# jinggqu/NextGen-UIA

Hardware: AMD Instinct MI355X
Metric: images/sec fwd+bwd BiomedCLIP+Mona bs=256 (higher is better)
Workload: dtype bf16

## Files before the change

nextgen-uia_amd/csrc/attention_bwd.hip:

```cpp
#include "uia_common.h"
#include "uia_kernels.h"

#ifdef ABWD_STAMPS
__device__ unsigned long long uia_abwd_stamps[8 * 8];
extern "C" int uia_abwd_read_stamps(unsigned long long* host) {
    return (int)hipMemcpyFromSymbol(host, HIP_SYMBOL(uia_abwd_stamps), sizeof(uia_abwd_stamps));
}
#define STAMP() __builtin_amdgcn_s_memtime()
#endif

namespace {

typedef __attribute__((ext_vector_type(4))) short s16x4;
typedef __attribute__((ext_vector_type(8))) short s16x8;

__device__ __forceinline__ void glds16(const char* gsrc, char* lds_wave_base) {
    const unsigned dst_u = __builtin_amdgcn_readfirstlane((unsigned)(uintptr_t)(__attribute__((address_space(3))) char*)lds_wave_base);
    unsigned keep;
    asm volatile("s_mov_b32 %0, m0\n\ts_mov_b32 m0, %2\n\ts_nop 0\n\tglobal_load_lds_dwordx4 %1, off\n\ts_mov_b32 m0, %0"
                 : "=&s"(keep) : "v"(gsrc), "s"(dst_u) : "memory");
}
__device__ __forceinline__ void glds4(const char* gsrc, char* lds_wave_base) {
    const unsigned dst_u = __builtin_amdgcn_readfirstlane((unsigned)(uintptr_t)(__attribute__((address_space(3))) char*)lds_wave_base);
    unsigned keep;
// ... 227 lines not shown
                qT[dt] = tr_pair(Qb + off, Qb + off + 16 * 128);
            }
        }
        const bool full_q = p.mask_kind == UIA_MASK_NONE && 32 * u + 32 <= L;
#pragma unroll
        for (int a = 0; a < KTW; ++a) {
            const int kt = wave + BWD_WAVES * a;
            if (kt < LT) {
                const int key = 16 * kt + li;
                bf16x8 pf, sf;
                f32x4 s[2], dp[2];
#pragma unroll
                for (int hq = 0; hq < 2; ++hq) {
                    s[hq] = mma(qf[hq][0], kf[a][0], f32x4{0.f, 0.f, 0.f, 0.f});
                    dp[hq] = mma(gf[hq][0], vf[a][0], f32x4{0.f, 0.f, 0.f, 0.f});
                }
#pragma unroll
                for (int hq = 0; hq < 2; ++hq) {
                    s[hq] = mma(qf[hq][1], kf[a][1], s[hq]);
                    dp[hq] = mma(gf[hq][1], vf[a][1], dp[hq]);
                }
#ifdef ABWD_NO_VALU
                if (true) {
#pragma unroll
                    for (int e = 0; e < 8; ++e) { pf[e] = (bf16_t)s[e >> 2][e & 3]; sf[e] = (bf16_t)dp[e >> 2][e & 3]; }
                } else
#endif
                if (full_q && 16 * kt + 16 <= L) {
#pragma unroll
                    for (int hq = 0; hq < 2; ++hq)
#pragma unroll
                        for (int r = 0; r < 4; ++r) {
                            const float pv = __builtin_amdgcn_exp2f(fmaf(s[hq][r], sc, -ls[hq][r]));
                            const float dsv = pv * fmaf(dp[hq][r], p.scale, -dl[hq][r]);
                            pf[4 * hq + r] = (bf16_t)pv;
                            sf[4 * hq + r] = (bf16_t)dsv;
                        }
                } else if (p.mask_kind != UIA_MASK_CAUSAL && 32 * u + 32 <= L) {
                    const bool key_ok = key < klen;
#pragma unroll
                    for (int hq = 0; hq < 2; ++hq)
#pragma unroll
                        for (int r = 0; r < 4; ++r) {
                            const float pe = __builtin_amdgcn_exp2f(fmaf(s[hq][r], sc, -ls[hq][r]));
                            const float pv = key_ok ? pe : 0.f;
                            const float dsv = pv * fmaf(dp[hq][r], p.scale, -dl[hq][r]);
                            pf[4 * hq + r] = (bf16_t)pv;
                            sf[4 * hq + r] = (bf16_t)dsv;
                        }
                } else {
#pragma unroll
                    for (int hq = 0; hq < 2; ++hq)
#pragma unroll
                        for (int r = 0; r < 4; ++r) {
                            const int qrow = 32 * u + 16 * hq + 4 * g + r;
                            const int kmax = p.mask_kind == UIA_MASK_CAUSAL ? (qrow < klen - 1 ? qrow : klen - 1) : klen - 1;
                            const bool ok = qrow < L && key <= kmax;
                            const float pv = ok ? __builtin_amdgcn_exp2f(fmaf(s[hq][r], sc, -ls[hq][r])) : 0.f;
                            const float dsv = pv * fmaf(dp[hq][r], p.scale, -dl[hq][r]);
                            pf[4 * hq + r] = (bf16_t)pv;
                            sf[4 * hq + r] = (bf16_t)dsv;
                        }
                }
                {
                    typedef __attribute__((ext_vector_type(4))) __bf16 bf16x4_t;
                    char* rowp = dST + key * 64;
                    const int sw = (key >> 1) & 7;
                    *(bf16x4_t*)(rowp + (((0 + g) ^ sw) << 3)) = bf16x4_t{sf[0], sf[1], sf[2], sf[3]};
                    *(bf16x4_t*)(rowp + (((4 + g) ^ sw) << 3)) = bf16x4_t{sf[4], sf[5], sf[6], sf[7]};
                }
#ifndef ABWD_NO_DVDK
#pragma unroll
                for (int dt = 0; dt < 4; ++dt) {
                    if constexpr (LAZY_T) {
                        const int off = trow * 128 + (((2 * dt + (pp >> 1)) ^ tsw) << 4) + 8 * (pp & 1);
                        gT[dt] = tr_pair(Gb + off, Gb + off + 16 * 128);
                        qT[dt] = tr_pair(Qb + off, Qb + off + 16 * 128);
                    }
                    dVt[a][dt] = __builtin_amdgcn_mfma_f32_16x16x32_bf16(gT[dt], pf, dVt[a][dt], 0, 0, 0);
                    dKt[a][dt] = __builtin_amdgcn_mfma_f32_16x16x32_bf16(qT[dt], sf, dKt[a][dt], 0, 0, 0);
                }
#endif
            }
        }
        }
#ifdef ABWD_STAMPS
        asm volatile("s_waitcnt lgkmcnt(0)" ::: "memory");
        const unsigned long long st3 = STAMP();
#endif
#ifndef ABWD_NO_DQ
        if (u > 0) {
#else
        if (false) {
#endif
            const int hq = wave >> 2, dt = wave & 3;
            f32x4 dq = f32x4{0.f, 0.f, 0.f, 0.f}, dq1 = f32x4{0.f, 0.f, 0.f, 0.f};
            const int ch = 2 * dt + (pp >> 1);
            const int c8 = 4 * hq + pp;
            auto dq_step = [&](int kbk, f32x4 accq) {
                const char* klo = Ks + (32 * kbk + nrow) * 128 + ((ch ^ nsw_lo) << 4) + 8 * (pp & 1);
                const char* khi = Ks + (32 * kbk + nrow + 4) * 128 + ((ch ^ nsw_hi) << 4) + 8 * (pp & 1);
                const char* slo = dSTr + (32 * kbk + nrow) * 64 + ((c8 ^ nsw_lo) << 3);
                const char* shi = dSTr + (32 * kbk + nrow + 4) * 64 + ((c8 ^ nsw_hi) << 3);
                return __builtin_amdgcn_mfma_f32_16x16x32_bf16(tr_pair(klo, khi), tr_pair(slo, shi), accq, 0, 0, 0);
            };
#pragma unroll 1
            for (int kbk = 0; kbk < NP; kbk += 2) {
                dq = dq_step(kbk, dq);
                if (kbk + 1 < NP) dq1 = dq_step(kbk + 1, dq1);
            }
            dq_hold = dq + dq1;
        }
#ifdef ABWD_STAMPS
        asm volatile("" :: "v"(dq_hold));
        const unsigned long long st4 = STAMP();
        st_acc[0] += st1 - st0; st_acc[1] += st2 - st1; st_acc[2] += st3 - st2; st_acc[3] += st4 - st3;
#endif
    }
#ifndef ABWD_NO_DQ
    store_dq(NP - 1);
#endif
#pragma unroll
    for (int a = 0; a < KTW; ++a) {
        const int kt = wave + BWD_WAVES * a;
        const int key = 16 * kt + li;
        if (kt < LT && key < L) {
            bf16_t* krow = (bf16_t*)p.dk + (row0 + key) * p.ld_dqkv + (size_t)h * 64 + 4 * g;
            bf16_t* vrow = (bf16_t*)p.dv + (row0 + key) * p.ld_dqkv + (size_t)h * 64 + 4 * g;
            const size_t kbo = ((size_t)(2 * h) * (size_t)p.dqkv_kb_rows + row0 + key) * 32 + 4 * g, kbp = (size_t)p.dqkv_kb_rows * 32;
#pragma unroll
            for (int dt = 0; dt < 4; ++dt) {
                store4(p.dqkv_kb_rows ? (bf16_t*)p.dk + kbo + (dt >> 1) * kbp + 16 * (dt & 1) : krow + 16 * dt, dKt[a][dt]);
                store4(p.dqkv_kb_rows ? (bf16_t*)p.dv + kbo + (dt >> 1) * kbp + 16 * (dt & 1) : vrow + 16 * dt, dVt[a][dt]);
            }
        }
    }
#ifdef ABWD_STAMPS
    if (blockIdx.x == 1500 && lane == 0) {
        unsigned long long* o = uia_abwd_stamps + wave * 8;
        o[0] = st_acc[0]; o[1] = st_acc[1]; o[2] = st_acc[2]; o[3] = st_acc[3]; o[4] = st_pro; o[5] = STAMP() - st_begin;
    }
#endif
}

struct ctrue { static constexpr bool value = true; };
struct cfalse { static constexpr bool value = false; };
template <int V> struct cint { static constexpr int value = V; };

#ifndef ABWD_ORDER17
#define ABWD_ORDER17 1
#endif
constexpr bool ORDER17 = ABWD_ORDER17 != 0;

template <int NW, bool VLDS, bool OLDS>
__global__ __launch_bounds__(64 * NW, (NW + 3) / 4) void attn_bwd_units_kernel(const UiaAttnParams p) {
    extern __shared__ __attribute__((aligned(16))) char smem[];
    constexpr int KVS = VLDS ? 4096 : 2048;
    constexpr bool KGLOBAL = false, QGLOBAL = false;
    const int L = p.L;
    const int LT = (L + 15) >> 4, NP = (LT + 1) >> 1;
    char* QGg = smem;
    char* KVg = QGg + LT * 4096;
    char* STg = KVg + LT * KVS;
    int* queue = (int*)(STg + LT * 128);
    char* OBg = STg + LT * 128 + 64;
    float* lseb = (float*)(OBg + LT * 2048);
    const lptr QG = (lptr)smem, KV = QG + LT * 4096, ST = KV + LT * KVS;

    const int tid = threadIdx.x, lane = tid & 63;
    const int wave = __builtin_amdgcn_readfirstlane(tid >> 6);
#ifdef ABWD_STAMPS
    const unsigned long long st_begin = STAMP();
    unsigned long long st_u[2] = {0, 0}, st_n[2] = {0, 0}, st_pro = 0, st_loop = 0, st_iter = 0;
#endif
    const int b = blockIdx.x / p.H, h = blockIdx.x - b * p.H;
    const size_t row0 = (size_t)b * L;
    const size_t rs = (size_t)p.ld_qkv * 2, rso = (size_t)p.lddo * 2, rsO = (size_t)p.ldo * 2;
    const char* qb = (const char*)p.q + (row0 * p.ld_qkv + (size_t)h * 64) * 2;
    const char* kb = (const char*)p.k + (row0 * p.ld_qkv + (size_t)h * 64) * 2;
    const char* vb = (const char*)p.v + (row0 * p.ld_qkv + (size_t)h * 64) * 2;
    const char* gb = (const char*)p.dout + (row0 * p.lddo + (size_t)h * 64) * 2;
    const char* ob = (const char*)p.out + (row0 * p.ldo + (size_t)h * 64) * 2;
    const int li = lane & 15, g = lane >> 4;
    int klen = L;
    if (p.mask_kind == UIA_MASK_KEYPAD && p.keylen) { klen = p.keylen[b]; klen = klen < 1 ? 1 : (klen > L ? L : klen); }
    klen = __builtin_amdgcn_readfirstlane(klen);
    const bool causal = p.mask_kind == UIA_MASK_CAUSAL;

    if constexpr (OLDS) {
        const int npieces = 2 * LT;
        for (int q = wave; q < npieces; q += NW) {
            const int r = 8 * q + (lane >> 3);
            const int gr = r < L ? r : L - 1;
            const int c = ((lane & 7) ^ (r & 6)) * 16;
            const int t = q >> 1, half = (q & 1) * 1024;
            glds16(gb + gr * rso + c, QGg + t * 4096 + 2048 + half);
            glds16(p.out_kb_rows ? (const char*)p.out + (((size_t)(2 * h + (c >> 6)) * (size_t)p.out_kb_rows + row0 + gr) << 6) + (c & 63) : ob + gr * rsO + c,
                   OBg + q * 1024);
        }
        for (int i = wave; i * 64 < 16 * LT; i += NW) {
            int r = 64 * i + lane;
            r = r < L ? r : L - 1;
            glds4((const char*)(p.lse + ((size_t)b * p.H + h) * L + r), (char*)(lseb + 64 * i));
        }
        for (int q = wave; q < npieces; q += NW) {
            const int r = 8 * q + (lane >> 3);
            const int gr = r < L ? r : L - 1;
            const int c = ((lane & 7) ^ (r & 6)) * 16;
            const int t = q >> 1, half = (q & 1) * 1024;
            glds16(kb + gr * rs + c, KVg + t * KVS + half);
            glds16(qb + gr * rs + c, QGg + t * 4096 + half);
            if (VLDS) glds16(vb + gr * rs + c, KVg + t * KVS + 2048 + half);
        }
        if (tid == 0) *queue = 0;
        const int nk = ((npieces - wave + NW - 1) / NW) * (VLDS ? 3 : 2);
        if (nk >= 9) asm volatile("s_waitcnt vmcnt(9)" ::: "memory");
        else if (nk >= 6) asm volatile("s_waitcnt vmcnt(6)" ::: "memory");
        else asm volatile("s_waitcnt vmcnt(0)" ::: "memory");
        __syncthreads();
        for (int r0 = 0; r0 < 16 * LT; r0 += NW * 8) {
            const int r = r0 + (tid >> 3), part = tid & 7;
            if (r < 16 * LT) {
                const int off = (r & 15) * 128 + ((part ^ (r & 6)) << 4);
                const bf16x8 gv = *(const bf16x8*)(QGg + (r >> 4) * 4096 + 2048 + off);
                const bf16x8 ovv = *(const bf16x8*)(OBg + (r >> 4) * 2048 + off);
                float d = 0.f;
#pragma unroll
                for (int e = 0; e < 8; ++e) d = fmaf((float)gv[e], (float)ovv[e], d);
                d += __builtin_bit_cast(float, __builtin_amdgcn_update_dpp(0, __builtin_bit_cast(int, d), 0xB1, 0xF, 0xF, false));
                d += __builtin_bit_cast(float, __builtin_amdgcn_update_dpp(0, __builtin_bit_cast(int, d), 0x4E, 0xF, 0xF, false));
                d += __builtin_bit_cast(float, __builtin_amdgcn_update_dpp(0, __builtin_bit_cast(int, d), 0x141, 0xF, 0xF, false));
                if (part == 0) {
                    float* st = (float*)(STg + (r >> 4) * 128) + (r & 15);
                    st[0] = r < L ? lseb[r] * 1.44269504088896341f : 0.f;
                    st[16] = r < L ? -d : 0.f;
                }
            }
        }
        asm volatile("s_waitcnt vmcnt(0)" ::: "memory");
        __syncthreads();
    } else
    {
        constexpr int RPP = NW * 8, MAXP = (288 + RPP - 1) / RPP;
        bf16x8 gv[MAXP], ov[MAXP];
        float lv[MAXP];
#pragma unroll
        for (int i = 0; i < MAXP; ++i) {
            const int r = i * RPP + (tid >> 3), part = tid & 7;
            if (i * RPP < 16 * LT) {
                const int gr = r < L ? r : L - 1;
                gv[i] = *(const bf16x8*)(gb + gr * rso + part * 16);
                ov[i] = *(const bf16x8*)(p.out_kb_rows ? (const char*)p.out + (((size_t)(2 * h + (part >> 2)) * (size_t)p.out_kb_rows + row0 + gr) << 6) + (part & 3) * 16
                                                       : ob + gr * rsO + part * 16);
                lv[i] = p.lse[((size_t)b * p.H + h) * L + gr];
            }
        }
        const int npieces = 2 * LT;
        for (int q = wave; q < npieces; q += NW) {
            const int r = 8 * q + (lane >> 3);
            const int gr = r < L ? r : L - 1;
            const int c = ((lane & 7) ^ (r & 6)) * 16;
            const int t = q >> 1, half = (q & 1) * 1024;
            glds16(kb + gr * rs + c, KVg + t * KVS + half);
            glds16(qb + gr * rs + c, QGg + t * 4096 + half);
            glds16(gb + gr * rso + c, QGg + t * 4096 + 2048 + half);
            if (VLDS) glds16(vb + gr * rs + c, KVg + t * KVS + 2048 + half);
        }
        if (tid == 0) *queue = 0;
#pragma unroll
        for (int i = 0; i < MAXP; ++i) {
            const int r = i * RPP + (tid >> 3), part = tid & 7;
            if (i * RPP < 16 * LT) {
                float d = 0.f;
#pragma unroll
                for (int e = 0; e < 8; ++e) d = fmaf((float)gv[i][e], (float)ov[i][e], d);
                d += __builtin_bit_cast(float, __builtin_amdgcn_update_dpp(0, __builtin_bit_cast(int, d), 0xB1, 0xF, 0xF, false));
                d += __builtin_bit_cast(float, __builtin_amdgcn_update_dpp(0, __builtin_bit_cast(int, d), 0x4E, 0xF, 0xF, false));
                d += __builtin_bit_cast(float, __builtin_amdgcn_update_dpp(0, __builtin_bit_cast(int, d), 0x141, 0xF, 0xF, false));
                if (part == 0 && r < 16 * LT) {
                    float* st = (float*)(STg + (r >> 4) * 128) + (r & 15);
                    st[0] = r < L ? lv[i] * 1.44269504088896341f : 0.f;
                    st[16] = r < L ? -d : 0.f;
                }
            }
        }
        asm volatile("s_waitcnt vmcnt(0)" ::: "memory");
        __syncthreads();
    }
#ifdef ABWD_STAMPS
    st_pro = STAMP() - st_begin;
#endif

    const float sc = p.scale * 1.44269504088896341f;
    const int offR0 = li * 128 + ((g ^ (li & 6)) << 4);
    const int offR1 = offR0 ^ 64;
    const int qq = li >> 2, pp = li & 3;
    const int trow = 4 * g + qq;
    const int tsw = trow & 6;
    int toff[4];
#pragma unroll
    for (int dt = 0; dt < 4; ++dt) toff[dt] = trow * 128 + (((2 * dt + (pp >> 1)) ^ tsw) << 4) + 8 * (pp & 1);
    const f32x4 zero4 = f32x4{0.f, 0.f, 0.f, 0.f};

    for (;;) {
        int unit = 0;
        if (lane == 0) unit = atomicAdd(queue, 1);
        unit = __builtin_amdgcn_readfirstlane(unit);
        if (unit >= 2 * LT) break;
#ifdef ABWD_STAMPS
        const unsigned long long st_u0 = STAMP();
#endif
        bool is_key = unit < LT;
        int tile = is_key ? unit : unit - LT;
        if (ORDER17 && LT == 17) {
            if (unit < 3) { is_key = true; tile = unit; }
            else if (unit < 10) { is_key = false; tile = unit - 3; }
            else if (unit < 24) { is_key = true; tile = unit - 7; }
            else { is_key = false; tile = unit - 17; }
        }
        if (is_key) {
            const int kt = tile;
#include "attention_bwd_key_unit.inc"
        } else {
            const int qt = tile;
#include "attention_bwd_qry_unit.inc"
        }
#ifdef ABWD_STAMPS
        st_u[is_key ? 0 : 1] += STAMP() - st_u0; st_n[is_key ? 0 : 1] += 1;
#endif
    }
#ifdef ABWD_STAMPS
    if (blockIdx.x == 1500 && lane == 0 && wave < 8) {
        unsigned long long* o = uia_abwd_stamps + wave * 8;
        o[0] = st_pro; o[1] = st_u[0]; o[2] = st_u[1]; o[3] = st_n[0]; o[4] = st_n[1]; o[5] = STAMP() - st_begin; o[6] = st_loop; o[7] = st_iter;
    }
#endif
}
template <int NW>
__global__ __launch_bounds__(64 * NW, 2) void attn_bwd_persist_kernel(const UiaAttnParams p, const int nheads) {
    extern __shared__ __attribute__((aligned(16))) char smem[];
    constexpr bool VLDS = true, KGLOBAL = true, QGLOBAL = true;
    constexpr int KVS = 4096;
    const int L = p.L;
    const int LT = (L + 15) >> 4, NP = (LT + 1) >> 1;
    char* QGg = smem;
    char* KVg = QGg + LT * 4096;
    char* STg = KVg + LT * KVS;
    char* OBg = STg + 2 * LT * 128;
    float* lseb = (float*)(OBg + LT * 2048);
    int* ctr = (int*)(lseb + ((16 * LT + 63) & ~63));
    const lptr QG = (lptr)smem, KV = QG + LT * 4096;
    const lptr STb = KV + LT * KVS;
    lptr ST = STb;

    const int tid = threadIdx.x, lane = tid & 63;
    const int wave = __builtin_amdgcn_readfirstlane(tid >> 6);
#ifdef ABWD_STAMPS
    const unsigned long long st_begin = STAMP();
    unsigned long long st_u[2] = {0, 0}, st_n[2] = {0, 0}, st_pro = 0, st_loop = 0, st_iter = 0, st_bar = 0;
#endif
    const int li = lane & 15, g = lane >> 4;
    const bool causal = p.mask_kind == UIA_MASK_CAUSAL;
    const size_t rs = (size_t)p.ld_qkv * 2, rso = (size_t)p.lddo * 2, rsO = (size_t)p.ldo * 2;
    const float sc = p.scale * 1.44269504088896341f;
    const int offR0 = li * 128 + ((g ^ (li & 6)) << 4);
    const int offR1 = offR0 ^ 64;
    const int qq = li >> 2, pp = li & 3;
    const int trow = 4 * g + qq;
    const int tsw = trow & 6;
    int toff[4];
#pragma unroll
    for (int dt = 0; dt < 4; ++dt) toff[dt] = trow * 128 + (((2 * dt + (pp >> 1)) ^ tsw) << 4) + 8 * (pp & 1);
    const f32x4 zero4 = f32x4{0.f, 0.f, 0.f, 0.f};

    int b = 0, h = 0, klen = L;
    size_t row0 = 0;
    const char *qb = nullptr, *kb = nullptr, *vb = nullptr, *gb = nullptr;
    auto set_head = [&](int n) {
        b = n / p.H; h = n - b * p.H;
        row0 = (size_t)b * L;
        qb = (const char*)p.q + (row0 * p.ld_qkv + (size_t)h * 64) * 2;
        kb = (const char*)p.k + (row0 * p.ld_qkv + (size_t)h * 64) * 2;
        vb = (const char*)p.v + (row0 * p.ld_qkv + (size_t)h * 64) * 2;
        gb = (const char*)p.dout + (row0 * p.lddo + (size_t)h * 64) * 2;
        klen = L;
        if (p.mask_kind == UIA_MASK_KEYPAD && p.keylen) { klen = p.keylen[b]; klen = klen < 1 ? 1 : (klen > L ? L : klen); }
        klen = __builtin_amdgcn_readfirstlane(klen);
    };
    auto stage_qg = [&](int n) {
        const int nb = n / p.H, nh = n - nb * p.H;
        const size_t nrow0 = (size_t)nb * L;
        const char* nq = (const char*)p.q + (nrow0 * p.ld_qkv + (size_t)nh * 64) * 2;
        const char* ng = (const char*)p.dout + (nrow0 * p.lddo + (size_t)nh * 64) * 2;
        const char* no = (const char*)p.out + (nrow0 * p.ldo + (size_t)nh * 64) * 2;
        for (int q = wave; q < 2 * LT; q += NW) {
            const int r = 8 * q + (lane >> 3);
            const int gr = r < L ? r : L - 1;
            const int c = ((lane & 7) ^ (r & 6)) * 16;
            const int t = q >> 1, half = (q & 1) * 1024;
            glds16(nq + gr * rs + c, QGg + t * 4096 + half);
            glds16(ng + gr * rso + c, QGg + t * 4096 + 2048 + half);
            glds16(p.out_kb_rows ? (const char*)p.out + (((size_t)(2 * nh + (c >> 6)) * (size_t)p.out_kb_rows + nrow0 + gr) << 6) + (c & 63) : no + gr * rsO + c,
                   OBg + q * 1024);
        }
        for (int i = wave; i * 64 < 16 * LT; i += NW) {
            int r = 64 * i + lane;
            r = r < L ? r : L - 1;
            glds4((const char*)(p.lse + ((size_t)nb * p.H + nh) * L + r), (char*)(lseb + 64 * i));
        }
    };
    auto stage_kv = [&]() {
        for (int q = wave; q < 2 * LT; q += NW) {
            const int r = 8 * q + (lane >> 3);
            const int gr = r < L ? r : L - 1;
            const int c = ((lane & 7) ^ (r & 6)) * 16;
            const int t = q >> 1, half = (q & 1) * 1024;
            glds16(kb + gr * rs + c, KVg + t * KVS + half);
            glds16(vb + gr * rs + c, KVg + t * KVS + 2048 + half);
        }
    };
    auto delta = [&](char* st_dst) {
        for (int r0 = 0; r0 < 16 * LT; r0 += NW * 8) {
            const int r = r0 + (tid >> 3), part = tid & 7;
            if (r < 16 * LT) {
                const int off = (r & 15) * 128 + ((part ^ (r & 6)) << 4);
                const bf16x8 gv = *(const bf16x8*)(QGg + (r >> 4) * 4096 + 2048 + off);
                const bf16x8 ovv = *(const bf16x8*)(OBg + (r >> 4) * 2048 + off);
                float d = 0.f;
#pragma unroll
                for (int e = 0; e < 8; ++e) d = fmaf((float)gv[e], (float)ovv[e], d);
                d += __builtin_bit_cast(float, __builtin_amdgcn_update_dpp(0, __builtin_bit_cast(int, d), 0xB1, 0xF, 0xF, false));
                d += __builtin_bit_cast(float, __builtin_amdgcn_update_dpp(0, __builtin_bit_cast(int, d), 0x4E, 0xF, 0xF, false));
                d += __builtin_bit_cast(float, __builtin_amdgcn_update_dpp(0, __builtin_bit_cast(int, d), 0x141, 0xF, 0xF, false));
                if (part == 0) {
                    float* st = (float*)(st_dst + (r >> 4) * 128) + (r & 15);
                    st[0] = r < L ? lseb[r] * 1.44269504088896341f : 0.f;
                    st[16] = r < L ? -d : 0.f;
                }
            }
        }
    };
    auto next_unit = [&](int which) {
        int u = 0;
        if (lane == 0) u = atomicAdd(ctr + which, 1);
        return __builtin_amdgcn_readfirstlane(u);
    };
    auto seam = [&]() {
        asm volatile("s_waitcnt vmcnt(0)" ::: "memory");
        __syncthreads();
    };

    int n = blockIdx.x;
    if (n >= nheads) return;
    stage_qg(n);
    if (tid == 0) { ctr[0] = 0; ctr[1] = 0; }
    seam();
    delta(STg);
    __syncthreads();
    set_head(n);
#ifdef ABWD_STAMPS
    st_pro = STAMP() - st_begin;
#endif
    int cur = 0;
    for (;;) {
        ST = STb + cur * (LT * 128);
        stage_kv();
        for (;;) {
            const int kt = next_unit(0);
            if (kt >= LT) break;
#ifdef ABWD_STAMPS
            const unsigned long long st_u0 = STAMP();
#endif
#include "attention_bwd_key_unit.inc"
// ... 28 lines not shown
#endif
        seam();
        delta(STg + (cur ^ 1) * (LT * 128));
        if (tid == 0) { ctr[0] = 0; ctr[1] = 0; }
        __syncthreads();
#ifdef ABWD_STAMPS
        st_bar += STAMP() - st_b1;
#endif
        n = nn;
        set_head(n);
        cur ^= 1;
    }
#ifdef ABWD_STAMPS
    if (blockIdx.x == 100 && lane == 0 && wave < 8) {
        unsigned long long* o = uia_abwd_stamps + wave * 8;
        o[0] = st_pro; o[1] = st_u[0]; o[2] = st_u[1]; o[3] = st_n[0]; o[4] = st_n[1]; o[5] = STAMP() - st_begin; o[6] = st_bar; o[7] = st_iter;
    }
#endif
}
__host__ __device__ constexpr int persist_lds_bytes(int LT) {
    return LT * 8192 + 2 * LT * 128 + LT * 2048 + ((16 * LT + 63) / 64) * 256 + 64 + 1024;
}
constexpr int PERSIST_LT_MAX = 15;

__host__ __device__ constexpr int units_lds_bytes(int LT, bool vlds, bool olds = false) {
    const int kvs = vlds ? 4096 : 2048, need = kvs + 64 - LT * 128;
    return LT * 4096 + LT * kvs + LT * 128 + 64 + (olds ? LT * 2048 + ((16 * LT + 63) / 64) * 256 + 1024 : (need > 1024 ? need : 1024));
}
constexpr int OLDS_LT_MAX = 15;


__global__ __launch_bounds__(256) void attn_bwd_f32_kernel(const UiaAttnParams p) {
    extern __shared__ __attribute__((aligned(16))) char smem[];
    const int L = p.L;
    float* A = (float*)smem;
    float* Bm = A + (size_t)L * 64;
    float* lse = Bm + (size_t)L * 64;
    float* delta = lse + L;
    const int tid = threadIdx.x;
    const int b = blockIdx.x / p.H, h = blockIdx.x - b * p.H;
    const size_t row0 = (size_t)b * L;
    const float* qb = (const float*)p.q + row0 * p.ld_qkv + (size_t)h * 64;
    const float* kb = (const float*)p.k + row0 * p.ld_qkv + (size_t)h * 64;
    const float* vb = (const float*)p.v + row0 * p.ld_qkv + (size_t)h * 64;
    const float* gb = (const float*)p.dout + row0 * p.lddo + (size_t)h * 64;
    const float* ob = (const float*)p.out + row0 * p.ldo + (size_t)h * 64;
    int klen = L;
    if (p.mask_kind == UIA_MASK_KEYPAD && p.keylen) { klen = p.keylen[b]; klen = klen < 1 ? 1 : (klen > L ? L : klen); }

    for (int r = tid; r < L; r += 256) {
        float d = 0.f;
        for (int c = 0; c < 64; ++c) d = fmaf(gb[(size_t)r * p.lddo + c], ob[(size_t)r * p.ldo + c], d);
        delta[r] = d;
        lse[r] = p.lse[((size_t)b * p.H + h) * L + r];
    }
    for (int i = tid; i < L * 16; i += 256) {
        const int r = i >> 4, c = (i & 15) * 4;
        *(f32x4*)(A + r * 64 + c) = *(const f32x4*)(kb + (size_t)r * p.ld_qkv + c);
        *(f32x4*)(Bm + r * 64 + c) = *(const f32x4*)(vb + (size_t)r * p.ld_qkv + c);
    }
    __syncthreads();
    for (int qi = tid; qi < L; qi += 256) {
        float q[64], go[64], dq[64];
#pragma unroll
        for (int c = 0; c < 64; ++c) { q[c] = qb[(size_t)qi * p.ld_qkv + c]; go[c] = gb[(size_t)qi * p.lddo + c]; dq[c] = 0.f; }
        const int kend = p.mask_kind == UIA_MASK_CAUSAL ? (qi + 1 < klen ? qi + 1 : klen) : klen;
        const float lq = lse[qi], dq_delta = delta[qi];
        for (int k = 0; k < kend; ++k) {
            float s = 0.f, dp = 0.f;
#pragma unroll
            for (int c = 0; c < 64; ++c) { s = fmaf(q[c], A[k * 64 + c], s); dp = fmaf(go[c], Bm[k * 64 + c], dp); }
            const float pv = expf(s * p.scale - lq);
            const float ds = pv * (dp - dq_delta) * p.scale;
#pragma unroll
            for (int c = 0; c < 64; ++c) dq[c] = fmaf(ds, A[k * 64 + c], dq[c]);
        }
        float* drow = (float*)p.dq + (row0 + qi) * p.ld_dqkv + (size_t)h * 64;
#pragma unroll
        for (int c = 0; c < 64; ++c) drow[c] = dq[c];
    }
    __syncthreads();
    for (int i = tid; i < L * 16; i += 256) {
        const int r = i >> 4, c = (i & 15) * 4;
        *(f32x4*)(A + r * 64 + c) = *(const f32x4*)(qb + (size_t)r * p.ld_qkv + c);
        *(f32x4*)(Bm + r * 64 + c) = *(const f32x4*)(gb + (size_t)r * p.lddo + c);
    }
    __syncthreads();
    for (int ki = tid; ki < L; ki += 256) {
        float kv[64], acc[64];
        float* vrow = (float*)p.dv + (row0 + ki) * p.ld_dqkv + (size_t)h * 64;
        float* krow = (float*)p.dk + (row0 + ki) * p.ld_dqkv + (size_t)h * 64;
        if (ki >= klen) {
#pragma unroll
            for (int c = 0; c < 64; ++c) { vrow[c] = 0.f; krow[c] = 0.f; }
            continue;
        }
        const int qstart = p.mask_kind == UIA_MASK_CAUSAL ? ki : 0;
#pragma unroll
        for (int c = 0; c < 64; ++c) { kv[c] = kb[(size_t)ki * p.ld_qkv + c]; acc[c] = 0.f; }
        for (int qi = qstart; qi < L; ++qi) {
            float s = 0.f;
#pragma unroll
            for (int c = 0; c < 64; ++c) s = fmaf(A[qi * 64 + c], kv[c], s);
            const float pv = expf(s * p.scale - lse[qi]);
#pragma unroll
            for (int c = 0; c < 64; ++c) acc[c] = fmaf(pv, Bm[qi * 64 + c], acc[c]);
        }
#pragma unroll
        for (int c = 0; c < 64; ++c) { vrow[c] = acc[c]; acc[c] = 0.f; }
        float vv[64];
#pragma unroll
        for (int c = 0; c < 64; ++c) vv[c] = vb[(size_t)ki * p.ld_qkv + c];
        for (int qi = qstart; qi < L; ++qi) {
            float s = 0.f, dp = 0.f;
#pragma unroll
            for (int c = 0; c < 64; ++c) { s = fmaf(A[qi * 64 + c], kv[c], s); dp = fmaf(Bm[qi * 64 + c], vv[c], dp); }
            const float pv = expf(s * p.scale - lse[qi]);
            const float ds = pv * (dp - delta[qi]) * p.scale;
#pragma unroll
            for (int c = 0; c < 64; ++c) acc[c] = fmaf(ds, A[qi * 64 + c], acc[c]);
        }
#pragma unroll
        for (int c = 0; c < 64; ++c) krow[c] = acc[c];
    }
}

template <int LT_MAX>
int launch_bf16(hipStream_t stream, const UiaAttnParams& p) {
    const int LT = (p.L + 15) / 16, NP = (LT + 1) / 2, LPK = NP * 32;
    const int lds = bwd_lds_bytes(LPK);
    auto kern = attn_bwd_bf16_kernel<LT_MAX>;
    static UiaDevOnce attr_once;
        constexpr int LPKM = ((LT_MAX + 1) / 2) * 32;
        static_assert(bwd_lds_bytes(LPKM) <= 160 * 1024, "LDS budget");
    UIA_ENSURE_LDS_ATTR(attr_once, kern, bwd_lds_bytes(LPKM));
    hipLaunchKernelGGL(kern, dim3(p.B * p.H), dim3(64 * BWD_WAVES), lds, stream, p);
    UIA_CHECK_LAUNCH();
    return 0;
}

template <int NW, bool VLDS, bool OLDS>
int launch_units(hipStream_t stream, const UiaAttnParams& p) {
    const int LT = (p.L + 15) / 16;
    auto kern = attn_bwd_units_kernel<NW, VLDS, OLDS>;
    static UiaDevOnce attr_once;
    constexpr int LTM = OLDS ? OLDS_LT_MAX : 18;
    static_assert(units_lds_bytes(LTM, true, OLDS) <= 160 * 1024, "LDS budget");
    UIA_ENSURE_LDS_ATTR(attr_once, kern, units_lds_bytes(LTM, VLDS, OLDS));
    hipLaunchKernelGGL(kern, dim3(p.B * p.H), dim3(64 * NW), units_lds_bytes(LT, VLDS, OLDS), stream, p);
    UIA_CHECK_LAUNCH();
    return 0;
}

int launch_persist(hipStream_t stream, const UiaAttnParams& p) {
    const int LT = (p.L + 15) / 16;
    auto kern = attn_bwd_persist_kernel<8>;
    static UiaDevOnce attr_once;
    static_assert(persist_lds_bytes(PERSIST_LT_MAX) <= 160 * 1024, "LDS budget");
    UIA_ENSURE_LDS_ATTR(attr_once, kern, persist_lds_bytes(PERSIST_LT_MAX));
    int dev = 0, ncu = 0;
    UIA_CHECK_HIP(hipGetDevice(&dev));
    UIA_CHECK_HIP(hipDeviceGetAttribute(&ncu, hipDeviceAttributeMultiprocessorCount, dev));
    const int nheads = p.B * p.H;
    int grid = nheads < ncu ? nheads : ncu;
    const int per = (nheads + grid - 1) / grid;
    grid = (nheads + per - 1) / per;
    hipLaunchKernelGGL(kern, dim3(grid), dim3(64 * 8), persist_lds_bytes(LT), stream, p, nheads);
    UIA_CHECK_LAUNCH();
    return 0;
}

}

int uia_attn_bwd_launch(hipStream_t stream, int dtype, const UiaAttnParams& p, int cfg) {
    UIA_CHECK_ARG(cfg >= 0 && cfg <= 7, "uia_attn_bwd: unknown kernel configuration %d", cfg);
    UIA_CHECK_ARG(dtype == UIA_BF16 || dtype == UIA_F32, "uia_attn_bwd: bad dtype %d", dtype);
    UIA_CHECK_ARG(p.B > 0 && p.H > 0 && p.L > 0, "uia_attn_bwd: empty problem");
    UIA_CHECK_ARG(p.scale > 0.f && p.scale < 3.0e38f, "uia_attn_bwd: scale must be positive and finite (matches the forward's lse), got %g", (double)p.scale);
    UIA_CHECK_ARG(!p.cu_seqlens, "uia_attn_bwd: packed sequences (cu_seqlens) are a forward-only layout");
    UIA_CHECK_ARG((p.out_kb_rows == 0 && p.dqkv_kb_rows == 0) ||
                  (p.dh == 64 && dtype == UIA_BF16 && (p.out_kb_rows == 0 || p.out_kb_rows >= (int64_t)p.B * p.L) && (p.dqkv_kb_rows == 0 || p.dqkv_kb_rows >= (int64_t)p.B * p.L)),
                  "uia_attn_bwd: K-blocked out / dq, dk, dv need the bf16 head-dim-64 path and at least B*L rows");
    if (p.dh != 64) return uia_attn_small_launch(stream, dtype, p, true);
    UIA_CHECK_ARG(p.q && p.k && p.v && p.out && p.dout && p.lse && p.dq && p.dk && p.dv, "uia_attn_bwd: null tensor");
    const int esz = dtype == UIA_BF16 ? 2 : 4;
    UIA_CHECK_ARG((p.ld_qkv * esz) % 16 == 0 && (p.ldo * esz) % 16 == 0 && (p.lddo * esz) % 16 == 0 && (p.ld_dqkv * esz) % 8 == 0,
                  "uia_attn_bwd: leading dimensions must keep 16-byte rows");
    UIA_CHECK_ARG(((uintptr_t)p.q | (uintptr_t)p.k | (uintptr_t)p.v | (uintptr_t)p.out | (uintptr_t)p.dout) % 16 == 0, "uia_attn_bwd: alignment");
    UIA_CHECK_ARG(((uintptr_t)p.dq | (uintptr_t)p.dk | (uintptr_t)p.dv) % 8 == 0, "uia_attn_bwd: output alignment");
    UIA_CHECK_ARG(p.mask_kind != UIA_MASK_KEYPAD || p.keylen, "uia_attn_bwd: key-padding mask needs keylen");
    if (dtype == UIA_F32) {
        UIA_CHECK_ARG(p.L <= 272, "uia_attn_bwd: L=%d exceeds 272", p.L);
        const int lds = (2 * p.L * 64 + 2 * p.L) * 4;
        static UiaDevOnce attr_once;
        UIA_ENSURE_LDS_ATTR(attr_once, attn_bwd_f32_kernel, (2 * 272 * 64 + 2 * 272) * 4);
        hipLaunchKernelGGL(attn_bwd_f32_kernel, dim3(p.B * p.H), dim3(256), lds, stream, p);
        UIA_CHECK_LAUNCH();
        return 0;
    }
    UIA_CHECK_ARG(p.L <= 288, "uia_attn_bwd: bf16 path keeps Q, K, dO of a head in LDS: L=%d exceeds 288", p.L);
    const int LT = (p.L + 15) / 16;
    if (cfg == 0) cfg = 2;
    if (cfg == 2) return LT <= OLDS_LT_MAX ? launch_units<8, true, true>(stream, p) : launch_units<8, true, false>(stream, p);
    if (cfg == 6) return launch_units<8, true, false>(stream, p);
    if (cfg == 7) return LT <= OLDS_LT_MAX ? launch_units<12, true, true>(stream, p) : launch_units<12, true, false>(stream, p);
    if (cfg == 3) return launch_units<4, false, false>(stream, p);
    if (cfg == 4) return launch_units<8, false, false>(stream, p);
    if (cfg == 5) {
        UIA_CHECK_ARG(LT <= PERSIST_LT_MAX, "uia_attn_bwd: the persistent kernel holds at most %d tokens (L = %d)", 16 * PERSIST_LT_MAX, p.L);
        return launch_persist(stream, p);
    }
    if (LT <= 8) return launch_bf16<8>(stream, p);
    if (LT <= 16) return launch_bf16<16>(stream, p);
    return launch_bf16<18>(stream, p);
}
```

Measured before the change: 6425.

## Add wide two-tile work units to attention backward for L=17 tiles

Adds a WIDE variant of the units kernel where each work unit handles two adjacent 16-row key or query tiles. This lets K/V or Q/dO fragments loaded from LDS be reused across two MFMA tiles, and halves the number of queue atomics and per-unit overheads. An odd trailing tile is handled by a single-tile unit. It becomes the default when LT==17 (BiomedCLIP's 197 tokens), at the cost of more registers per wave and fewer, larger units for load balancing.

```diff
diff --git a/nextgen-uia_amd/csrc/attention_bwd.hip b/nextgen-uia_amd/csrc/attention_bwd.hip
--- a/nextgen-uia_amd/csrc/attention_bwd.hip
+++ b/nextgen-uia_amd/csrc/attention_bwd.hip
@@ -403,7 +403,7 @@
 #endif
 constexpr bool ORDER17 = ABWD_ORDER17 != 0;
 
-template <int NW, bool VLDS, bool OLDS>
+template <int NW, bool VLDS, bool OLDS, bool WIDE = false>
 __global__ __launch_bounds__(64 * NW, (NW + 3) / 4) void attn_bwd_units_kernel(const UiaAttnParams p) {
     extern __shared__ __attribute__((aligned(16))) char smem[];
     constexpr int KVS = VLDS ? 4096 : 2048;
@@ -432,7 +432,7 @@
     const char* vb = (const char*)p.v + (row0 * p.ld_qkv + (size_t)h * 64) * 2;
     const char* gb = (const char*)p.dout + (row0 * p.lddo + (size_t)h * 64) * 2;
     const char* ob = (const char*)p.out + (row0 * p.ldo + (size_t)h * 64) * 2;
-    const int li = lane & 15, g = lane >> 4;
+    int li = lane & 15, g = lane >> 4;
     int klen = L;
     if (p.mask_kind == UIA_MASK_KEYPAD && p.keylen) { klen = p.keylen[b]; klen = klen < 1 ? 1 : (klen > L ? L : klen); }
     klen = __builtin_amdgcn_readfirstlane(klen);
@@ -543,8 +543,8 @@
 #endif
 
     const float sc = p.scale * 1.44269504088896341f;
-    const int offR0 = li * 128 + ((g ^ (li & 6)) << 4);
-    const int offR1 = offR0 ^ 64;
+    int offR0 = li * 128 + ((g ^ (li & 6)) << 4);
+    int offR1 = offR0 ^ 64;
     const int qq = li >> 2, pp = li & 3;
     const int trow = 4 * g + qq;
     const int tsw = trow & 6;
@@ -557,19 +557,36 @@
         int unit = 0;
         if (lane == 0) unit = atomicAdd(queue, 1);
         unit = __builtin_amdgcn_readfirstlane(unit);
-        if (unit >= 2 * LT) break;
+        if (unit >= (WIDE ? 2 * NP : 2 * LT)) break;
 #ifdef ABWD_STAMPS
         const unsigned long long st_u0 = STAMP();
 #endif
-        bool is_key = unit < LT;
+        bool is_key = unit < LT, wide = false;
         int tile = is_key ? unit : unit - LT;
-        if (ORDER17 && LT == 17) {
+        if constexpr (WIDE) {
+            asm volatile("" : "+v"(li), "+v"(g), "+v"(offR0), "+v"(offR1), "+v"(toff[0]), "+v"(toff[1]), "+v"(toff[2]), "+v"(toff[3]));
+            const int NPR = LT >> 1;
+            wide = unit < 2 * NPR;
+            is_key = wide ? unit < NPR : unit == 2 * NPR;
+            tile = wide ? 2 * (is_key ? unit : unit - NPR) : LT - 1;
+            asm volatile("" : "+s"(tile));
+        } else if (ORDER17 && LT == 17) {
             if (unit < 3) { is_key = true; tile = unit; }
             else if (unit < 10) { is_key = false; tile = unit - 3; }
             else if (unit < 24) { is_key = true; tile = unit - 7; }
             else { is_key = false; tile = unit - 17; }
         }
-        if (is_key) {
+        if (wide) {
+            if constexpr (WIDE) {
+                if (is_key) {
+                    const int kt0 = tile;
+#include "attention_bwd_key_unit_wide.inc"
+                } else {
+                    const int qt0 = tile;
+#include "attention_bwd_qry_unit_wide.inc"
+                }
+            }
+        } else if (is_key) {
             const int kt = tile;
 #include "attention_bwd_key_unit.inc"
         } else {
@@ -904,6 +921,19 @@
     return 0;
 }
 
+template <bool OLDS>
+int launch_wide(hipStream_t stream, const UiaAttnParams& p) {
+    const int LT = (p.L + 15) / 16;
+    auto kern = attn_bwd_units_kernel<8, true, OLDS, true>;
+    static UiaDevOnce attr_once;
+    constexpr int LTM = OLDS ? OLDS_LT_MAX : 18;
+    static_assert(units_lds_bytes(LTM, true, OLDS) <= 160 * 1024, "LDS budget");
+    UIA_ENSURE_LDS_ATTR(attr_once, kern, units_lds_bytes(LTM, true, OLDS));
+    hipLaunchKernelGGL(kern, dim3(p.B * p.H), dim3(64 * 8), units_lds_bytes(LT, true, OLDS), stream, p);
+    UIA_CHECK_LAUNCH();
+    return 0;
+}
+
 int launch_persist(hipStream_t stream, const UiaAttnParams& p) {
     const int LT = (p.L + 15) / 16;
     auto kern = attn_bwd_persist_kernel<8>;
@@ -925,7 +955,7 @@
 }
 
 int uia_attn_bwd_launch(hipStream_t stream, int dtype, const UiaAttnParams& p, int cfg) {
-    UIA_CHECK_ARG(cfg >= 0 && cfg <= 7, "uia_attn_bwd: unknown kernel configuration %d", cfg);
+    UIA_CHECK_ARG(cfg >= 0 && cfg <= 8, "uia_attn_bwd: unknown kernel configuration %d", cfg);
     UIA_CHECK_ARG(dtype == UIA_BF16 || dtype == UIA_F32, "uia_attn_bwd: bad dtype %d", dtype);
     UIA_CHECK_ARG(p.B > 0 && p.H > 0 && p.L > 0, "uia_attn_bwd: empty problem");
     UIA_CHECK_ARG(p.scale > 0.f && p.scale < 3.0e38f, "uia_attn_bwd: scale must be positive and finite (matches the forward's lse), got %g", (double)p.scale);
@@ -952,7 +982,8 @@
     }
     UIA_CHECK_ARG(p.L <= 288, "uia_attn_bwd: bf16 path keeps Q, K, dO of a head in LDS: L=%d exceeds 288", p.L);
     const int LT = (p.L + 15) / 16;
-    if (cfg == 0) cfg = 2;
+    if (cfg == 0) cfg = LT == 17 ? 8 : 2;
+    if (cfg == 8) return LT <= OLDS_LT_MAX ? launch_wide<true>(stream, p) : launch_wide<false>(stream, p);
     if (cfg == 2) return LT <= OLDS_LT_MAX ? launch_units<8, true, true>(stream, p) : launch_units<8, true, false>(stream, p);
     if (cfg == 6) return launch_units<8, true, false>(stream, p);
     if (cfg == 7) return LT <= OLDS_LT_MAX ? launch_units<12, true, true>(stream, p) : launch_units<12, true, false>(stream, p);
diff --git a/nextgen-uia_amd/csrc/attention_bwd_key_unit_wide.inc b/nextgen-uia_amd/csrc/attention_bwd_key_unit_wide.inc
--- /dev/null
+++ b/nextgen-uia_amd/csrc/attention_bwd_key_unit_wide.inc
@@ -0,0 +1,148 @@
+{
+            const int kt1 = kt0 + 1;
+            const int key0 = 16 * kt0 + li, key1 = key0 + 16;
+            uint4 kf[2][2], vf[2][2];
+#pragma unroll
+            for (int a = 0; a < 2; ++a) {
+                kf[a][0] = lds_u4(KV + (kt0 + a) * KVS + offR0);
+                kf[a][1] = lds_u4(KV + (kt0 + a) * KVS + offR1);
+                vf[a][0] = lds_u4(KV + (kt0 + a) * KVS + 2048 + offR0);
+                vf[a][1] = lds_u4(KV + (kt0 + a) * KVS + 2048 + offR1);
+            }
+            f32x4 dVt[2][4], dKt[2][4];
+#pragma unroll
+            for (int a = 0; a < 2; ++a)
+#pragma unroll
+                for (int dt = 0; dt < 4; ++dt) { dVt[a][dt] = zero4; dKt[a][dt] = zero4; }
+            const int ub_lo = 16 * kt0 >= klen ? NP : (causal ? kt0 >> 1 : 0);
+            const bool key_ok0 = key0 < klen, key_ok1 = key1 < klen;
+            lptr r0 = QG + ub_lo * 8192 + offR0;
+            lptr r1 = QG + ub_lo * 8192 + offR1;
+            lptr tp0 = QG + ub_lo * 8192 + toff[0];
+            lptr tp1 = QG + ub_lo * 8192 + toff[1];
+            lptr tp2 = QG + ub_lo * 8192 + toff[2];
+            lptr tp3 = QG + ub_lo * 8192 + toff[3];
+            lptr sp = ST + ub_lo * 256 + 16 * g;
+            asm volatile("" : "+v"(r0), "+v"(r1), "+v"(tp0), "+v"(tp1), "+v"(tp2), "+v"(tp3), "+v"(sp));
+            uint4 qf[2][2], gf[2][2];
+            f32x4 ls[2], dl[2], s[2][2], dp[2][2];
+            auto load_rows = [&](int ahead) {
+                qf[0][0] = lds_u4(r0 + ahead);        gf[0][0] = lds_u4(r0 + ahead + 2048);
+                qf[0][1] = lds_u4(r1 + ahead);        gf[0][1] = lds_u4(r1 + ahead + 2048);
+                qf[1][0] = lds_u4(r0 + ahead + 4096); gf[1][0] = lds_u4(r0 + ahead + 6144);
+                qf[1][1] = lds_u4(r1 + ahead + 4096); gf[1][1] = lds_u4(r1 + ahead + 6144);
+            };
+            auto load_stats = [&](int ahead) {
+                ls[0] = lds_f4(sp + ahead); ls[1] = lds_f4(sp + ahead + 128);
+                dl[0] = lds_f4(sp + ahead + 64); dl[1] = lds_f4(sp + ahead + 192);
+            };
+            auto products = [&](int a, int nq) {
+#pragma unroll
+                for (int hq = 0; hq < nq; ++hq) {
+                    s[a][hq] = mma(qf[hq][0], kf[a][0], zero4);   dp[a][hq] = mma(gf[hq][0], vf[a][0], dl[hq]);
+                    s[a][hq] = mma(qf[hq][1], kf[a][1], s[a][hq]); dp[a][hq] = mma(gf[hq][1], vf[a][1], dp[a][hq]);
+                }
+            };
+            auto key_block = [&](auto kind_c, int ub) {
+                constexpr int KIND = decltype(kind_c)::value;
+                constexpr int HI = KIND == 2 ? 0 : 4096;
+                constexpr int NQ = KIND == 2 ? 1 : 2;
+                constexpr int VK = KIND == 0 ? 4 : 7;
+                const int nxt = ub + 1 < NP ? 1 : 0;
+                bf16x8 gT[4], qT[4];
+                qT[0] = tr_pair(tp0, tp0 + HI); gT[0] = tr_pair(tp0 + 2048, tp0 + 2048 + HI);
+                qT[1] = tr_pair(tp1, tp1 + HI); gT[1] = tr_pair(tp1 + 2048, tp1 + 2048 + HI);
+                qT[2] = tr_pair(tp2, tp2 + HI); gT[2] = tr_pair(tp2 + 2048, tp2 + 2048 + HI);
+                qT[3] = tr_pair(tp3, tp3 + HI); gT[3] = tr_pair(tp3 + 2048, tp3 + 2048 + HI);
+                bf16x8 pf[2], sf[2];
+                auto softmax = [&](int a) {
+                    const int key = a ? key1 : key0;
+                    const bool key_ok = a ? key_ok1 : key_ok0;
+#pragma unroll
+                    for (int hq = 0; hq < NQ; ++hq)
+#pragma unroll
+                        for (int r = 0; r < 4; ++r) {
+                            float pv = __builtin_amdgcn_exp2f(fmaf(s[a][hq][r], sc, -ls[hq][r]));
+                            float dsv = pv * dp[a][hq][r];
+                            if constexpr (KIND != 0) {
+                                const int qrow = 32 * ub + 16 * hq + 4 * g + r;
+                                const bool ok = qrow < L && key_ok && (!causal || key <= qrow);
+                                pv = ok ? pv : 0.f;
+                                dsv = ok ? dsv : 0.f;
+                            }
+                            pf[a][4 * hq + r] = (bf16_t)pv;
+                            sf[a][4 * hq + r] = (bf16_t)dsv;
+                        }
+                    if constexpr (NQ == 1) {
+#pragma unroll
+                        for (int e = 4; e < 8; ++e) { pf[a][e] = (bf16_t)0.f; sf[a][e] = (bf16_t)0.f; }
+                    }
+                };
+                __builtin_amdgcn_sched_barrier(0);
+                products(0, NQ);
+                products(1, NQ);
+                softmax(0);
+                __builtin_amdgcn_sched_group_barrier(0x008, 4 * NQ, 0);
+#pragma unroll
+                for (int i = 0; i < 4 * NQ; ++i) {
+                    __builtin_amdgcn_sched_group_barrier(0x008, 1, 0);
+                    __builtin_amdgcn_sched_group_barrier(0x002, VK, 0);
+                }
+                __builtin_amdgcn_sched_barrier(0);
+                load_rows(8192 * nxt);
+#pragma unroll
+                for (int dt = 0; dt < 4; ++dt) {
+                    dVt[0][dt] = __builtin_amdgcn_mfma_f32_16x16x32_bf16(gT[dt], pf[0], dVt[0][dt], 0, 0, 0);
+                    dKt[0][dt] = __builtin_amdgcn_mfma_f32_16x16x32_bf16(qT[dt], sf[0], dKt[0][dt], 0, 0, 0);
+                }
+                softmax(1);
+#pragma unroll
+                for (int i = 0; i < 8; ++i) {
+                    __builtin_amdgcn_sched_group_barrier(0x008, 1, 0);
+                    __builtin_amdgcn_sched_group_barrier(0x002, VK * NQ / 2, 0);
+                }
+                __builtin_amdgcn_sched_barrier(0);
+                load_stats(256 * nxt);
+#pragma unroll
+                for (int dt = 0; dt < 4; ++dt) {
+                    dVt[1][dt] = __builtin_amdgcn_mfma_f32_16x16x32_bf16(gT[dt], pf[1], dVt[1][dt], 0, 0, 0);
+                    dKt[1][dt] = __builtin_amdgcn_mfma_f32_16x16x32_bf16(qT[dt], sf[1], dKt[1][dt], 0, 0, 0);
+                }
+                __builtin_amdgcn_sched_barrier(0);
+                r0 += 8192; r1 += 8192; tp0 += 8192; tp1 += 8192; tp2 += 8192; tp3 += 8192; sp += 256;
+            };
+            if (ub_lo < NP) {
+                const int last = NP - 1, nfull = LT >> 1;
+                int f0 = causal ? (16 * kt1 + 46) >> 5 : 0, f1 = L >> 5;
+                f0 = f0 < ub_lo ? ub_lo : f0;
+                f1 = f1 > nfull ? nfull : f1;
+                if (16 * kt1 + 16 > klen || f0 > f1) { f0 = nfull; f1 = nfull; }
+                load_rows(0); load_stats(0);
+                int ub = ub_lo;
+#pragma unroll 1
+                for (; ub < f0 && ub < last; ++ub) key_block(cint<1>{}, ub);
+#pragma unroll 1
+                for (; ub < f1 && ub < last; ++ub) key_block(cint<0>{}, ub);
+#pragma unroll 1
+                for (; ub < last; ++ub) key_block(cint<1>{}, ub);
+                if (LT & 1) key_block(cint<2>{}, last);
+                else if (last >= f0 && last < f1) key_block(cint<0>{}, last);
+                else key_block(cint<1>{}, last);
+            }
+            int key_st = key0;
+            asm volatile("" : "+v"(key_st));
+#pragma unroll
+            for (int a = 0; a < 2; ++a) {
+                const int key = key_st + 16 * a;
+                if (key < L) {
+                    bf16_t* krow = (bf16_t*)p.dk + (row0 + key) * p.ld_dqkv + (size_t)h * 64 + 4 * g;
+                    bf16_t* vrow = (bf16_t*)p.dv + (row0 + key) * p.ld_dqkv + (size_t)h * 64 + 4 * g;
+                    const size_t kbo = ((size_t)(2 * h) * (size_t)p.dqkv_kb_rows + row0 + key) * 32 + 4 * g, kbp = (size_t)p.dqkv_kb_rows * 32;
+#pragma unroll
+                    for (int dt = 0; dt < 4; ++dt) {
+                        store4(p.dqkv_kb_rows ? (bf16_t*)p.dk + kbo + (dt >> 1) * kbp + 16 * (dt & 1) : krow + 16 * dt, dKt[a][dt] * p.scale);
+                        store4(p.dqkv_kb_rows ? (bf16_t*)p.dv + kbo + (dt >> 1) * kbp + 16 * (dt & 1) : vrow + 16 * dt, dVt[a][dt]);
+                    }
+                }
+            }
+}
diff --git a/nextgen-uia_amd/csrc/attention_bwd_qry_unit_wide.inc b/nextgen-uia_amd/csrc/attention_bwd_qry_unit_wide.inc
--- /dev/null
+++ b/nextgen-uia_amd/csrc/attention_bwd_qry_unit_wide.inc
@@ -0,0 +1,128 @@
+{
+            const int qrow0 = 16 * qt0 + li, qrow1 = qrow0 + 16;
+            uint4 qf[2][2], gf[2][2];
+            float lq[2];
+            f32x4 nd4[2];
+#pragma unroll
+            for (int i = 0; i < 2; ++i) {
+                qf[i][0] = lds_u4(QG + (qt0 + i) * 4096 + offR0);        qf[i][1] = lds_u4(QG + (qt0 + i) * 4096 + offR1);
+                gf[i][0] = lds_u4(QG + (qt0 + i) * 4096 + 2048 + offR0); gf[i][1] = lds_u4(QG + (qt0 + i) * 4096 + 2048 + offR1);
+                lq[i] = lds_f1(ST + (qt0 + i) * 128 + 4 * li);
+                const float nd = lds_f1(ST + (qt0 + i) * 128 + 64 + 4 * li);
+                nd4[i] = f32x4{nd, nd, nd, nd};
+            }
+            f32x4 dQt[2][4];
+#pragma unroll
+            for (int i = 0; i < 2; ++i)
+#pragma unroll
+                for (int dt = 0; dt < 4; ++dt) dQt[i][dt] = zero4;
+            int kend = klen;
+            if (causal && 16 * qt0 + 32 < kend) kend = 16 * qt0 + 32;
+            const int KB = (kend + 31) >> 5;
+            lptr r0 = KV + offR0;
+            lptr r1 = KV + offR1;
+            lptr tp0 = KV + toff[0];
+            lptr tp1 = KV + toff[1];
+            lptr tp2 = KV + toff[2];
+            lptr tp3 = KV + toff[3];
+            asm volatile("" : "+v"(r0), "+v"(r1), "+v"(tp0), "+v"(tp1), "+v"(tp2), "+v"(tp3));
+            uint4 ka[2][2], va[2][2];
+            f32x4 s[2][2], dp[2][2];
+            auto load_kv = [&](int ahead) {
+                ka[0][0] = lds_u4(r0 + ahead);       ka[0][1] = lds_u4(r1 + ahead);
+                ka[1][0] = lds_u4(r0 + ahead + KVS); ka[1][1] = lds_u4(r1 + ahead + KVS);
+                va[0][0] = lds_u4(r0 + ahead + 2048);       va[0][1] = lds_u4(r1 + ahead + 2048);
+                va[1][0] = lds_u4(r0 + ahead + KVS + 2048); va[1][1] = lds_u4(r1 + ahead + KVS + 2048);
+            };
+            auto products = [&](int hk) {
+#pragma unroll
+                for (int i = 0; i < 2; ++i) {
+                    s[hk][i] = mma(ka[hk][0], qf[i][0], zero4);    dp[hk][i] = mma(va[hk][0], gf[i][0], nd4[i]);
+                    s[hk][i] = mma(ka[hk][1], qf[i][1], s[hk][i]); dp[hk][i] = mma(va[hk][1], gf[i][1], dp[hk][i]);
+                }
+            };
+            auto qry_block = [&](auto kind_c, int kbk) {
+                constexpr int KIND = decltype(kind_c)::value;
+                constexpr int HI = KIND == 2 ? 0 : KVS;
+                constexpr int VK = KIND == 0 ? 4 : 6;
+                const int nxt = kbk + 1 < KB ? 1 : 0;
+                bf16x8 kT[4];
+                kT[0] = tr_pair(tp0, tp0 + HI); kT[1] = tr_pair(tp1, tp1 + HI);
+                kT[2] = tr_pair(tp2, tp2 + HI); kT[3] = tr_pair(tp3, tp3 + HI);
+                bf16x8 sf[2];
+                auto softmax = [&](int hk, int i) {
+                    const int qrow = i ? qrow1 : qrow0;
+#pragma unroll
+                    for (int r = 0; r < 4; ++r) {
+                        const float pv = __builtin_amdgcn_exp2f(fmaf(s[hk][i][r], sc, -lq[i]));
+                        float dsv = pv * dp[hk][i][r];
+                        if constexpr (KIND != 0) {
+                            const int keyv = 32 * kbk + 16 * hk + 4 * g + r;
+                            const bool ok = keyv < klen && (!causal || keyv <= qrow);
+                            dsv = ok ? dsv : 0.f;
+                        }
+                        sf[i][4 * hk + r] = (bf16_t)dsv;
+                    }
+                };
+                __builtin_amdgcn_sched_barrier(0);
+                products(0);
+                if constexpr (KIND != 2) products(1);
+                softmax(0, 0); softmax(0, 1);
+                if constexpr (KIND == 2) {
+#pragma unroll
+                    for (int e = 4; e < 8; ++e) { sf[0][e] = (bf16_t)0.f; sf[1][e] = (bf16_t)0.f; }
+                } else {
+                    softmax(1, 0);
+                    __builtin_amdgcn_sched_group_barrier(0x008, 8, 0);
+#pragma unroll
+                    for (int i = 0; i < 8; ++i) {
+                        __builtin_amdgcn_sched_group_barrier(0x008, 1, 0);
+                        __builtin_amdgcn_sched_group_barrier(0x002, VK, 0);
+                    }
+                }
+                __builtin_amdgcn_sched_barrier(0);
+                load_kv(2 * KVS * nxt);
+#pragma unroll
+                for (int dt = 0; dt < 4; ++dt) dQt[0][dt] = __builtin_amdgcn_mfma_f32_16x16x32_bf16(kT[dt], sf[0], dQt[0][dt], 0, 0, 0);
+                if constexpr (KIND != 2) {
+                    softmax(1, 1);
+#pragma unroll
+                    for (int i = 0; i < 4; ++i) {
+                        __builtin_amdgcn_sched_group_barrier(0x008, 1, 0);
+                        __builtin_amdgcn_sched_group_barrier(0x002, VK, 0);
+                    }
+                }
+                __builtin_amdgcn_sched_barrier(0);
+#pragma unroll
+                for (int dt = 0; dt < 4; ++dt) dQt[1][dt] = __builtin_amdgcn_mfma_f32_16x16x32_bf16(kT[dt], sf[1], dQt[1][dt], 0, 0, 0);
+                __builtin_amdgcn_sched_barrier(0);
+                r0 += 2 * KVS; r1 += 2 * KVS; tp0 += 2 * KVS; tp1 += 2 * KVS; tp2 += 2 * KVS; tp3 += 2 * KVS;
+            };
+            {
+                const int last = KB - 1;
+                const bool tail_last = 2 * last + 1 >= LT;
+                int f1 = causal ? (16 * qt0 + 1) >> 5 : klen >> 5;
+                f1 = f1 > (klen >> 5) ? klen >> 5 : f1;
+                f1 = f1 > (LT >> 1) ? LT >> 1 : f1;
+                load_kv(0);
+                int kbk = 0;
+#pragma unroll 1
+                for (; kbk < f1 && kbk < last; ++kbk) qry_block(cint<0>{}, kbk);
+#pragma unroll 1
+                for (; kbk < last; ++kbk) qry_block(cint<1>{}, kbk);
+                if (tail_last) qry_block(cint<2>{}, last);
+                else if (last < f1) qry_block(cint<0>{}, last);
+                else qry_block(cint<1>{}, last);
+            }
+#pragma unroll
+            for (int i = 0; i < 2; ++i) {
+                const int qrow = i ? qrow1 : qrow0;
+                if (qrow < L) {
+                    bf16_t* drow = (bf16_t*)p.dq + (row0 + qrow) * p.ld_dqkv + (size_t)h * 64 + 4 * g;
+                    const size_t kbo = ((size_t)(2 * h) * (size_t)p.dqkv_kb_rows + row0 + qrow) * 32 + 4 * g, kbp = (size_t)p.dqkv_kb_rows * 32;
+#pragma unroll
+                    for (int dt = 0; dt < 4; ++dt)
+                        store4(p.dqkv_kb_rows ? (bf16_t*)p.dq + kbo + (dt >> 1) * kbp + 16 * (dt & 1) : drow + 16 * dt, dQt[i][dt] * p.scale);
+                }
+            }
+}
```

Result: no change. 6431 (median of 6 runs) (+0.1%).
